# MarvelMathesh/sincformer-metacog-speech-enhancement

Hardware: AMD Instinct MI355X
Metric: audio frames/sec/GPU (16 kHz, 512-frame utts) + mask RMSE vs CPU ref (higher is better)
Workload: dtype fp16 MFMA operands (PerceptionAgent, fusion, Conformer GEMMs, heads) + bf16 attention core, fp32 accumulate (ops.POLICIES['mixed']); 1 GPU; B256 x 512-frame utterances (L40880, T512) forward; batch_per_gpu=256, samples=40880, frames_per_utt=512, launch=eager launches, streams=2, precision_policy=mixed

## Files before the change

sincformer_metacog_speech_enhancement_amd/csrc/conv16p.hip:

```cpp
#include "gemm16_epi.h"

struct ConvPParams {
  Gemm2Params g;
  Gemm2Params gs;
  const u16* x1; const float* sc1; const float* sh1;
  const u16* x2; const float* sc2; const float* sh2;
  int Lin, Cin, pad, nMt;
  long long x_batch_stride;
};

__device__ __forceinline__ float gelu_as(float z) {
  const float ax = fabsf(z) * 0.70710678118654752440f;
  const float t = __builtin_amdgcn_rcpf(1.0f + 0.3275911f * ax);
  const float ex = __builtin_amdgcn_exp2f(-0.72134752044448170368f * z * z);
  const float poly = t * (0.254829592f + t * (-0.284496736f + t * (1.421413741f + t * (-1.453152027f + t * 1.061405429f))));
  const float erfa = 1.0f - poly * ex;
  return z * (0.5f + 0.5f * copysignf(erfa, z));
}

typedef _Float16 h2_t __attribute__((ext_vector_type(2)));
__device__ __forceinline__ uint32_t gelu_as_h2p(uint32_t zb) {
  const h2_t z = __builtin_bit_cast(h2_t, zb);
  const h2_t az = __builtin_bit_cast(h2_t, zb & 0x7fff7fffu);
  const h2_t u = az * (h2_t)(_Float16)(0.3275911f * 0.70710678118654752440f) + (h2_t)(_Float16)1.0f;
  h2_t t;
  t[0] = __builtin_amdgcn_rcph(u[0]);
  t[1] = __builtin_amdgcn_rcph(u[1]);
  const h2_t ex = __builtin_elementwise_exp2(z * z * (h2_t)(_Float16)(-0.72134752044448170368f));
  h2_t poly = t * (_Float16)1.061405429f + (_Float16)(-1.453152027f);
  poly = poly * t + (_Float16)1.421413741f;
  poly = poly * t + (_Float16)(-0.284496736f);
  poly = poly * t + (_Float16)0.254829592f;
  poly = poly * t;
  const h2_t erfa = (h2_t)(_Float16)1.0f - poly * ex;
  const h2_t sg = __builtin_bit_cast(h2_t, (__builtin_bit_cast(uint32_t, erfa) & 0x7fff7fffu) | (zb & 0x80008000u));
  return __builtin_bit_cast(uint32_t, z * (sg * (_Float16)0.5f + (_Float16)0.5f));
}

template <class T, bool FULL>
__device__ __forceinline__ void convp_epilogue_impl(const Gemm2Params& g, f32x16 (&acc)[2][2], unsigned char* img, const float* bias_s,
                                                    int lane, int b, int colb, int row_base) {
  constexpr int ROWB = 144;
  const int l31 = lane & 31, hl = lane >> 5;
  float ps[2][4], pq[2][4];
#pragma unroll
  for (int j = 0; j < 2; ++j)
#pragma unroll
    for (int gq = 0; gq < 4; ++gq) {
      const int n0 = colb + j * 32 + 8 * gq + 4 * hl;
      const f32x4 bv = *reinterpret_cast<const f32x4*>(bias_s + n0);
      float s_ = 0.f, q_ = 0.f;
#pragma unroll
      for (int i = 0; i < 2; ++i) {
        const bool rowok = FULL || (row_base + i * 32 + l31 < g.Lout);
#pragma unroll
        for (int e = 0; e < 4; ++e) {
          const float v = acc[i][j][4 * gq + e] + bv[e];
          acc[i][j][4 * gq + e] = v;
          if (rowok) {
            s_ += v;
            q_ = __builtin_fmaf(v, v, q_);
          }
        }
      }
      ps[j][gq] = s_;
      pq[j][gq] = q_;
    }
  if (g.gn_partial) {
    const int cpg = g.gn_group >> 3;
    const int ngroups = g.N / g.gn_group;
    float v16[16];
#pragma unroll
    for (int j = 0; j < 2; ++j)
#pragma unroll
      for (int gq = 0; gq < 4; ++gq) {
        v16[j * 4 + gq] = ps[j][gq];
        v16[8 + j * 4 + gq] = pq[j][gq];
      }
    float tot = wave_sum16_transpose(v16, lane);
    if (cpg >= 2) tot += dpp_perm<0xB1>(tot);
    if (cpg == 4) tot += dpp_perm<0x4E>(tot);
    const int gq_ = lane & 3, j_ = (lane >> 2) & 1, stat = (lane >> 3) & 1;
    if (lane < 16 && (gq_ & (cpg - 1)) == 0 && (row_base >> 6) < g.gn_slots) {
      const long long sl = ((long long)b * g.gn_slots + (row_base >> 6)) * ngroups + (colb + j_ * 32 + 8 * gq_) / g.gn_group;
      g.gn_partial[sl * 2 + stat] = tot;
    }
  }
  const int osz = g.out_f32 == 1 ? 4 : 2;
  auto ors = __builtin_amdgcn_make_buffer_rsrc((void*)(reinterpret_cast<unsigned char*>(g.out) + (long long)b * g.o_batch_stride * osz), 0,
                                               g.Lout * g.ldo * osz, 0x00020000);
  if (g.out_f32 != 1) {
    __builtin_amdgcn_s_waitcnt(0xC07F);
    __builtin_amdgcn_wave_barrier();
#define CONVP_PACK_IMG(PK)                                                                                             \
  _Pragma("unroll") for (int i = 0; i < 2; ++i)                                                                        \
  _Pragma("unroll") for (int j = 0; j < 2; ++j)                                                                        \
  _Pragma("unroll") for (int gq = 0; gq < 4; ++gq) {                                                                   \
    u32x2 w;                                                                                                           \
    w[0] = PK(acc[i][j][4 * gq + 0], acc[i][j][4 * gq + 1]);                                                           \
    w[1] = PK(acc[i][j][4 * gq + 2], acc[i][j][4 * gq + 3]);                                                           \
    *reinterpret_cast<u32x2*>(img + (i * 32 + l31) * ROWB + (j * 32 + 8 * gq + 4 * hl) * 2) = w;                       \
  }
    if ((g.out_f32 == 2) == (T::id == SFM_DT_BF16)) { CONVP_PACK_IMG(F16::pack) } else { CONVP_PACK_IMG(BF16::pack) }
#undef CONVP_PACK_IMG
    __builtin_amdgcn_s_waitcnt(0xC07F);
    __builtin_amdgcn_wave_barrier();
    u32x4 rv[8];
#pragma unroll
    for (int k = 0; k < 8; ++k) {
      const int c = lane + 64 * k;
      rv[k] = *reinterpret_cast<const u32x4*>(img + (c >> 3) * ROWB + (c & 7) * 16);
    }
#pragma unroll
    for (int k = 0; k < 8; ++k) {
      const int c = lane + 64 * k;
      const int row = c >> 3, ch = c & 7;
      __builtin_amdgcn_raw_buffer_store_b128(rv[k], ors, ((row_base + row) * g.ldo + colb + ch * 8) * 2, 0, 0);
    }
  } else {
#pragma unroll
    for (int i = 0; i < 2; ++i) {
      __builtin_amdgcn_s_waitcnt(0xC07F);
      __builtin_amdgcn_wave_barrier();
#pragma unroll
      for (int j = 0; j < 2; ++j)
#pragma unroll
        for (int gq = 0; gq < 4; ++gq)
          *reinterpret_cast<f32x4*>(img + l31 * 272 + (j * 32 + 8 * gq + 4 * hl) * 4) =
              f32x4{acc[i][j][4 * gq + 0], acc[i][j][4 * gq + 1], acc[i][j][4 * gq + 2], acc[i][j][4 * gq + 3]};
      __builtin_amdgcn_s_waitcnt(0xC07F);
      __builtin_amdgcn_wave_barrier();
#pragma unroll
      for (int k = 0; k < 8; ++k) {
        const int c = lane + 64 * k;
        const int row = c >> 4, ch = c & 15;
        const u32x4 v = *reinterpret_cast<const u32x4*>(img + row * 272 + ch * 16);
        __builtin_amdgcn_raw_buffer_store_b128(v, ors, ((row_base + i * 32 + row) * g.ldo + colb + ch * 4) * 4, 0, 0);
      }
    }
  }
}

template <class T>
__device__ __forceinline__ void convp_epilogue(const Gemm2Params& g, f32x16 (&acc)[2][2], unsigned char* img, const float* bias_s,
                                               int lane, int b, int colb, int row_base) {
  if (row_base + 64 <= g.Lout) convp_epilogue_impl<T, true>(g, acc, img, bias_s, lane, b, colb, row_base);
  else convp_epilogue_impl<T, false>(g, acc, img, bias_s, lane, b, colb, row_base);
}

template <class T, int KS, int STRIDE, int NPASS, bool SKIP, bool TWO_IN>
__global__ __launch_bounds__(256, 2) void conv16p_kernel(ConvPParams p) {
  constexpr int R = 127 * STRIDE + KS;
  constexpr int PLANES = (STRIDE == 2 && KS > 1) ? 2 : 1;
  constexpr int PR = (((STRIDE == 2) ? (R + 1) / 2 : R) + 7) / 8 * 8;
  constexpr int PATCH = PLANES * PR * 128;
  constexpr int WT = 128 * 128;
  constexpr int TPS = NPASS * KS + (SKIP ? 1 : 0);
  static_assert(!SKIP || NPASS == 1, "the fused skip conv needs N = 128");
  static_assert(PATCH + 2 * WT >= 4 * 9216, "epilogue images fit in the patch + ring area");
  extern __shared__ __attribute__((aligned(16))) unsigned char smem[];
  unsigned char* ring = smem + PATCH;
  constexpr int RING = (TWO_IN && PATCH > 2 * WT) ? PATCH : 2 * WT;
  float* bias_s = reinterpret_cast<float*>(smem + PATCH + RING);

  const int tid = threadIdx.x, lane = tid & 63;
  const int wave = __builtin_amdgcn_readfirstlane(tid >> 6);
  const int wm = wave >> 1, wn = wave & 1;
  const int l31 = lane & 31, hl = lane >> 5;

  for (int i = tid; i < NPASS * 128; i += 256) bias_s[i] = p.g.bias ? p.g.bias[i] : 0.f;
  if (SKIP && tid < 128) bias_s[256 + tid] = p.gs.bias ? p.gs.bias[tid] : 0.f;
  int id = blockIdx.x;
  {
    const int total = gridDim.x, q = total >> 3, r = total & 7, xcd = id & 7, slot = id >> 3;
    id = (xcd < r ? xcd * (q + 1) : r * (q + 1) + (xcd - r) * q) + slot;
  }
  const int mtile = id % p.nMt, b = id / p.nMt;
  const int l0 = mtile * 128;
  const int nslab = p.Cin >> 6;
  const int Q = nslab * TPS;

  auto w_rs = __builtin_amdgcn_make_buffer_rsrc((void*)p.g.W, 0, p.g.w_records, 0x00020000);
  auto ws_rs = __builtin_amdgcn_make_buffer_rsrc((void*)(SKIP ? p.gs.W : p.g.W), 0, SKIP ? p.gs.w_records : p.g.w_records, 0x00020000);
  int b_row[4], b_swz[4];
#pragma unroll
  for (int i = 0; i < 4; ++i) {
    b_row[i] = (wave * 4 + i) * 8 + (lane >> 3);
    b_swz[i] = ((lane & 7) ^ ((b_row[i] >> 1) & 7)) * 8;
  }
  auto issue_w = [&](int q) {
    const int slab = q / TPS, j = q - slab * TPS;
    unsigned char* dst = ring + (q & 1) * WT;
    if (SKIP && j == TPS - 1) {
#pragma unroll
      for (int i = 0; i < 4; ++i)
        __builtin_amdgcn_raw_ptr_buffer_load_lds(ws_rs, (lds_ptr_t)(dst + (wave * 4 + i) * 1024), 16,
                                                 (b_row[i] * p.gs.Kpad + slab * 64 + b_swz[i]) * 2, 0, 0, 0);
    } else {
      const int np = j / KS, t = j - np * KS;
      const int koff = t * p.Cin + slab * 64;
#pragma unroll
      for (int i = 0; i < 4; ++i)
        __builtin_amdgcn_raw_ptr_buffer_load_lds(w_rs, (lds_ptr_t)(dst + (wave * 4 + i) * 1024), 16,
                                                 ((np * 128 + b_row[i]) * p.g.Kpad + koff + b_swz[i]) * 2, 0, 0, 0);
    }
  };

  f32x16 acc[NPASS][2][2], accs[2][2];
#pragma unroll
  for (int n = 0; n < NPASS; ++n)
#pragma unroll
    for (int i = 0; i < 2; ++i)
#pragma unroll
      for (int j = 0; j < 2; ++j)
#pragma unroll
        for (int r = 0; r < 16; ++r) acc[n][i][j][r] = 0.f;
#pragma unroll
  for (int i = 0; i < 2; ++i)
#pragma unroll
    for (int j = 0; j < 2; ++j)
#pragma unroll
      for (int r = 0; r < 16; ++r) accs[i][j][r] = 0.f;

  int fb_off[2][4];
#pragma unroll
  for (int j = 0; j < 2; ++j) {
    const int row = wn * 64 + j * 32 + l31;
#pragma unroll
    for (int s = 0; s < 4; ++s) fb_off[j][s] = row * 128 + (((2 * s + hl) ^ ((row >> 1) & 7)) << 4);
  }

  constexpr int JSTEP = (PLANES == 1 && STRIDE == 2) ? 2 : 1;
  constexpr int LROWS = PLANES * PR;
  constexpr int NPIECE = (LROWS + 7) / 8;
  auto x1_rs = __builtin_amdgcn_make_buffer_rsrc((void*)(p.x1 + (long long)b * p.x_batch_stride), 0, p.Lin * p.Cin * 2, 0x00020000);
  auto x2_rs = __builtin_amdgcn_make_buffer_rsrc((void*)((TWO_IN ? p.x2 : p.x1) + (long long)b * p.x_batch_stride), 0,
                                                 p.Lin * p.Cin * 2, 0x00020000);
  auto row_pos = [&](int lr) {
    const int plane = (PLANES == 2) ? (lr >= PR ? 1 : 0) : 0;
    const int idx = lr - plane * PR;
    const int j = (PLANES == 2) ? 2 * idx + plane : idx * JSTEP;
    const int pos = l0 * STRIDE - p.pad + j;
    return (lr < LROWS && j < R && pos >= 0 && pos < p.Lin) ? pos : -1;
  };
  const int sp_ = tid & 7, srow = tid >> 3;
  const int sc_ = sp_ ^ ((srow >> 1) & 7);
  auto stage_patch = [&](int slab) {
    for (int pc = wave; pc < NPIECE; pc += 4) {
      const int lr = pc * 8 + (lane >> 3);
      const int pos = row_pos(lr);
      const int c = (lane & 7) ^ ((lr >> 1) & 7);
      const int voff = pos >= 0 ? (pos * p.Cin + slab * 64 + c * 8) * 2 : -1;
      __builtin_amdgcn_raw_ptr_buffer_load_lds(x1_rs, (lds_ptr_t)(smem + pc * 1024), 16, voff, 0, 0, 0);
      if (TWO_IN) __builtin_amdgcn_raw_ptr_buffer_load_lds(x2_rs, (lds_ptr_t)(ring + pc * 1024), 16, voff, 0, 0, 0);
    }
    const int ch0 = slab * 64 + sc_ * 8;
    float a1[8], d1[8], a2[8];
    {
      const f32x4* ps = reinterpret_cast<const f32x4*>(p.sc1 + (long long)b * p.Cin + ch0);
      const f32x4* ph = reinterpret_cast<const f32x4*>(p.sh1 + (long long)b * p.Cin + ch0);
      const f32x4 s0 = ps[0], s1 = ps[1], h0 = ph[0], h1 = ph[1];
#pragma unroll
      for (int e = 0; e < 4; ++e) { a1[e] = s0[e]; a1[4 + e] = s1[e]; d1[e] = h0[e]; d1[4 + e] = h1[e]; }
      if (TWO_IN) {
        const f32x4* qs = reinterpret_cast<const f32x4*>(p.sc2 + (long long)b * p.Cin + ch0);
        const f32x4* qh = reinterpret_cast<const f32x4*>(p.sh2 + (long long)b * p.Cin + ch0);
        const f32x4 t0 = qs[0], t1 = qs[1], g0 = qh[0], g1 = qh[1];
#pragma unroll
        for (int e = 0; e < 4; ++e) { a2[e] = t0[e]; a2[4 + e] = t1[e]; d1[e] += g0[e]; d1[4 + e] += g1[e]; }
      }
    }
    wait_vmcnt<0>();
    __syncthreads();
#pragma unroll 2
    for (int lr = srow; lr < LROWS; lr += 32) {
      if (row_pos(lr) < 0) continue;
      unsigned char* q1 = smem + lr * 128 + sp_ * 16;
      const u32x4 v1 = *reinterpret_cast<const u32x4*>(q1);
      u32x4 v2 = {0u, 0u, 0u, 0u};
      if (TWO_IN) v2 = *reinterpret_cast<const u32x4*>(ring + lr * 128 + sp_ * 16);
      u32x4 o;
#pragma unroll
      for (int e = 0; e < 4; ++e) {
        if (T::id == SFM_DT_F16) {
          uint32_t zpk;
          float t0 = d1[2 * e], t1 = d1[2 * e + 1];
          if (TWO_IN) {
            asm("v_fma_mix_f32 %0, %1, %2, %3 op_sel:[0,0,0] op_sel_hi:[1,0,0]" : "=v"(t0) : "v"(v2[e]), "v"(a2[2 * e]), "v"(d1[2 * e]));
            asm("v_fma_mix_f32 %0, %1, %2, %3 op_sel:[1,0,0] op_sel_hi:[1,0,0]" : "=v"(t1) : "v"(v2[e]), "v"(a2[2 * e + 1]), "v"(d1[2 * e + 1]));
          }
          asm("v_fma_mixlo_f16 %0, %1, %2, %3 op_sel:[0,0,0] op_sel_hi:[1,0,0]\n\t"
              "v_fma_mixhi_f16 %0, %1, %4, %5 op_sel:[1,0,0] op_sel_hi:[1,0,0]"
              : "=&v"(zpk) : "v"(v1[e]), "v"(a1[2 * e]), "v"(t0), "v"(a1[2 * e + 1]), "v"(t1));
          o[e] = gelu_as_h2p(zpk);
          continue;
        }
        float z0 = T::to_f32((u16)(v1[e] & 0xffffu)) * a1[2 * e] + d1[2 * e];
        float z1 = T::to_f32((u16)(v1[e] >> 16)) * a1[2 * e + 1] + d1[2 * e + 1];
        if (TWO_IN) {
          z0 += T::to_f32((u16)(v2[e] & 0xffffu)) * a2[2 * e];
          z1 += T::to_f32((u16)(v2[e] >> 16)) * a2[2 * e + 1];
        }
        o[e] = pack2<T>(gelu_as(z0), gelu_as(z1));
      }
      *reinterpret_cast<u32x4*>(q1) = o;
    }
  };

  auto mma_tile = [&](int q, int t, f32x16 (&a)[2][2]) {
    const unsigned char* wb = ring + (q & 1) * WT;
    int arow[2];
#pragma unroll
    for (int i = 0; i < 2; ++i) {
      const int rw = wm * 64 + i * 32 + l31;
      arow[i] = (PLANES == 2) ? (t & 1) * PR + rw + (t >> 1) : ((STRIDE == 2) ? rw : rw + t);
    }
#pragma unroll
    for (int s = 0; s < 4; ++s) {
      u32x4 fa[2], fb[2];
#pragma unroll
      for (int i = 0; i < 2; ++i)
        fa[i] = *reinterpret_cast<const u32x4*>(smem + arow[i] * 128 + (((2 * s + hl) ^ ((arow[i] >> 1) & 7)) << 4));
#pragma unroll
      for (int j = 0; j < 2; ++j) fb[j] = *reinterpret_cast<const u32x4*>(wb + fb_off[j][s]);
#pragma unroll
      for (int i = 0; i < 2; ++i)
#pragma unroll
        for (int j = 0; j < 2; ++j) a[i][j] = T::mfma(fb[j], fa[i], a[i][j]);
    }
  };

  if (!TWO_IN) issue_w(0);
  for (int slab = 0; slab < nslab; ++slab) {
    if (slab > 0) __syncthreads();
    stage_patch(slab);
    __syncthreads();
    const int q0 = slab * TPS;
    if (TWO_IN) issue_w(q0);
#pragma unroll
    for (int j = 0; j < TPS; ++j) {
      const int q = q0 + j;
      wait_ring<0>();
      __builtin_amdgcn_s_barrier();
      if (j + 1 < TPS) issue_w(q + 1);
      if (SKIP && j == TPS - 1) {
        mma_tile(q, p.pad, accs);
      } else {
        const int np = j / KS, t = j - np * KS;
        if (np == 0) mma_tile(q, t, acc[0]);
        else mma_tile(q, t, acc[NPASS - 1]);
      }
      if (j + 1 == TPS && !TWO_IN && q + 1 < Q) issue_w(q + 1);
    }
  }
  __syncthreads();
  unsigned char* img = smem + wave * 9216;
#pragma unroll
  for (int n = 0; n < NPASS; ++n) convp_epilogue<T>(p.g, acc[n], img, bias_s, lane, b, n * 128 + wn * 64, l0 + wm * 64);
  if (SKIP) convp_epilogue<T>(p.gs, accs, img, bias_s + 256, lane, b, wn * 64, l0 + wm * 64);
}

template <class T, int KS, int STRIDE, int NPASS, bool SKIP, bool TWO_IN>
static int launch_convp(const ConvPParams& p, hipStream_t stream) {
  constexpr int R = 127 * STRIDE + KS;
  constexpr int PLANES = (STRIDE == 2 && KS > 1) ? 2 : 1;
  constexpr int PR = (((STRIDE == 2) ? (R + 1) / 2 : R) + 7) / 8 * 8;
  constexpr int patch = PLANES * PR * 128;
  constexpr int lds = patch + ((TWO_IN && patch > 2 * 128 * 128) ? patch : 2 * 128 * 128) + 384 * 4;
  SFM_LAUNCH_LDS((conv16p_kernel<T, KS, STRIDE, NPASS, SKIP, TWO_IN>), dim3(p.nMt * p.g.B), dim3(256), lds, stream, p);
  return SFM_OK;
}

static void convp_fill(Gemm2Params& g, const void* W, const float* bias, void* out, float* gn_partial, int B, int Lout, int N,
                       int Kpad, int out_f32, int gn_group) {
  g = Gemm2Params{};
  g.W = (const u16*)W; g.bias = bias; g.out = out; g.gn_partial = gn_partial;
  g.B = B; g.Lout = Lout; g.N = N; g.Npad = N; g.K = Kpad; g.Kpad = Kpad; g.ldo = N; g.o_batch_stride = (long long)Lout * N;
  g.alpha = 1.0f; g.epi = EPI_NONE; g.out_f32 = out_f32; g.gn_group = gn_group; g.nsplit = 0;
  g.w_records = (int)((long long)N * Kpad * 2);
  g.gn_slots = 2 * ((Lout + 127) / 128);
  const int osz = out_f32 == 1 ? 4 : 2;
  g.vec_ok = ((((uintptr_t)out) % 16) == 0 && ((N * osz) % 16) == 0) ? 1 : 0;
  g.p_drop = 0.f; g.seed = 0u; g.aux = nullptr; g.out2 = nullptr; g.resid = nullptr;
}

extern "C" int sfm_conv16p(const void* x1, const float* sc1, const float* sh1, const void* x2, const float* sc2, const float* sh2,
                           const void* W, const float* bias, void* out, float* gn_partial, const void* Ws, const float* bias_s,
                           void* out_s, float* gn_partial_s, int B, int Lin, int Cin, int N, int ksize, int stride, int pad,
                           int out_f32, int gn_group, int dtype, void* stream) {
  if (!x1 || !sc1 || !sh1 || !W || !out) return SFM_ERR_ARG;
  if ((x2 != nullptr) != (sc2 != nullptr) || (x2 != nullptr) != (sh2 != nullptr)) return SFM_ERR_ARG;
  if (B <= 0 || Lin <= 0 || Cin <= 0 || (Cin % 64) != 0 || (N != 128 && N != 256)) return SFM_ERR_SHAPE;
  if (out_f32 < 0 || out_f32 > 2) return SFM_ERR_SHAPE;
  if (gn_partial && gn_group != 8 && gn_group != 16 && gn_group != 32) return SFM_ERR_SHAPE;
  if ((long long)Lin * Cin * 2 >= (1LL << 31) || (long long)N * ksize * Cin * 2 >= (1LL << 31)) return SFM_ERR_SHAPE;
  if ((long long)((Lin + 2 * pad - ksize) / stride + 1) * N * 4 >= (1LL << 31)) return SFM_ERR_SHAPE;
  const int Lout = (Lin + 2 * pad - ksize) / stride + 1;
  if (Lout <= 0) return SFM_ERR_SHAPE;
  const bool skip = Ws != nullptr;
  if (skip && (!out_s || N != 128 || ksize != 7 || stride != 2)) return SFM_ERR_SHAPE;
  if ((((uintptr_t)out) % 16) != 0 || (out_s && (((uintptr_t)out_s) % 16) != 0)) return SFM_ERR_SHAPE;
  ConvPParams p{};
  convp_fill(p.g, W, bias, out, gn_partial, B, Lout, N, ksize * Cin, out_f32, gn_group);
  if (skip) convp_fill(p.gs, Ws, bias_s, out_s, gn_partial_s, B, Lout, N, Cin, out_f32, gn_group);
  p.x1 = (const u16*)x1; p.sc1 = sc1; p.sh1 = sh1; p.x2 = (const u16*)x2; p.sc2 = sc2; p.sh2 = sh2;
  p.Lin = Lin; p.Cin = Cin; p.pad = pad; p.nMt = (Lout + 127) / 128; p.x_batch_stride = (long long)Lin * Cin;
  hipStream_t st = (hipStream_t)stream;
  const bool two = x2 != nullptr;
  const int key = ksize * 100 + stride * 10 + pad;
#define CONVP_GO(TT)                                                                                       \
  if (key == 723 && N == 128 && skip) return two ? launch_convp<TT, 7, 2, 1, true, true>(p, st) : launch_convp<TT, 7, 2, 1, true, false>(p, st); \
  if (key == 723 && N == 256 && !skip && two) return launch_convp<TT, 7, 2, 2, false, true>(p, st);        \
  if (key == 311 && N == 128 && !two) return launch_convp<TT, 3, 1, 1, false, false>(p, st);                \
  if (key == 311 && N == 256 && !two) return launch_convp<TT, 3, 1, 2, false, false>(p, st);                \
  if (key == 522 && N == 256 && two) return launch_convp<TT, 5, 2, 2, false, true>(p, st);                  \
  if (key == 120 && N == 256 && two) return launch_convp<TT, 1, 2, 2, false, true>(p, st);
  if (dtype == SFM_DT_BF16) { CONVP_GO(BF16) }
  if (dtype == SFM_DT_F16) { CONVP_GO(F16) }
#undef CONVP_GO
  return SFM_ERR_SHAPE;
}
```

sincformer_metacog_speech_enhancement_amd/csrc/sfm_common.h:

```cpp
#pragma once
#include <hip/hip_runtime.h>
#include <stdint.h>
#include <atomic>
#include <mutex>
#include "sincformer_hip.h"

typedef uint16_t u16;
typedef __attribute__((ext_vector_type(4))) float f32x4;
typedef __attribute__((ext_vector_type(16))) float f32x16;
typedef __attribute__((ext_vector_type(8))) __bf16 bf16x8_t;
typedef __attribute__((ext_vector_type(8))) _Float16 f16x8_t;
typedef __attribute__((ext_vector_type(4))) short s16x4;
typedef __attribute__((ext_vector_type(4))) uint32_t u32x4;
typedef __attribute__((ext_vector_type(2))) uint32_t u32x2;
typedef __attribute__((ext_vector_type(2))) float f32x2;
typedef __attribute__((ext_vector_type(2))) __bf16 bf16x2_t;
typedef __attribute__((ext_vector_type(2))) _Float16 f16x2_t;

struct BF16 {
  static constexpr int id = SFM_DT_BF16;
  static __device__ __forceinline__ u16 from_f32(float f) {
    __bf16 h = (__bf16)f;
    return __builtin_bit_cast(u16, h);
  }
  static __device__ __forceinline__ float to_f32(u16 b) {
    return __builtin_bit_cast(float, (uint32_t)b << 16);
  }
  static __device__ __forceinline__ uint32_t pack(float lo, float hi) {
    f32x2 v = {lo, hi};
    return __builtin_bit_cast(uint32_t, __builtin_convertvector(v, bf16x2_t));
  }
  static __device__ __forceinline__ f32x16 mfma(u32x4 a, u32x4 b, f32x16 c) {
    return __builtin_amdgcn_mfma_f32_32x32x16_bf16(__builtin_bit_cast(bf16x8_t, a),
                                                   __builtin_bit_cast(bf16x8_t, b), c, 0, 0, 0);
  }
  static __device__ __forceinline__ f32x4 mfma16(u32x4 a, u32x4 b, f32x4 c) {
    return __builtin_amdgcn_mfma_f32_16x16x32_bf16(__builtin_bit_cast(bf16x8_t, a),
                                                   __builtin_bit_cast(bf16x8_t, b), c, 0, 0, 0);
  }
};

struct F16 {
  static constexpr int id = SFM_DT_F16;
  static __device__ __forceinline__ u16 from_f32(float f) {
    _Float16 h = (_Float16)f;
    return __builtin_bit_cast(u16, h);
  }
  static __device__ __forceinline__ float to_f32(u16 b) {
    return (float)__builtin_bit_cast(_Float16, b);
  }
  static __device__ __forceinline__ uint32_t pack(float lo, float hi) {
    f32x2 v = {lo, hi};
    return __builtin_bit_cast(uint32_t, __builtin_convertvector(v, f16x2_t));
  }
  static __device__ __forceinline__ f32x16 mfma(u32x4 a, u32x4 b, f32x16 c) {
    return __builtin_amdgcn_mfma_f32_32x32x16_f16(__builtin_bit_cast(f16x8_t, a),
                                                  __builtin_bit_cast(f16x8_t, b), c, 0, 0, 0);
  }
  static __device__ __forceinline__ f32x4 mfma16(u32x4 a, u32x4 b, f32x4 c) {
    return __builtin_amdgcn_mfma_f32_16x16x32_f16(__builtin_bit_cast(f16x8_t, a),
                                                  __builtin_bit_cast(f16x8_t, b), c, 0, 0, 0);
  }
};

template <class T>
__device__ __forceinline__ uint32_t pack2(float lo, float hi) {
  return T::pack(lo, hi);
}
template <class T>
__device__ __forceinline__ uint32_t pack2_out(float lo, float hi, bool other) {
  if (T::id == SFM_DT_BF16) return other ? F16::pack(lo, hi) : BF16::pack(lo, hi);
  return other ? BF16::pack(lo, hi) : F16::pack(lo, hi);
}

__device__ __forceinline__ uint32_t sfm_hash(uint32_t seed, unsigned long long idx) {
  uint32_t x = (uint32_t)idx * 0x9E3779B1u ^ (uint32_t)(idx >> 32) * 0x85EBCA77u ^ seed;
  x ^= x >> 16; x *= 0x7FEB352Du; x ^= x >> 15; x *= 0x846CA68Bu; x ^= x >> 16;
  return x;
}
__device__ __forceinline__ uint32_t sfm_keep_threshold(float p) { return (uint32_t)ceilf(p * 16777216.0f); }
__device__ __forceinline__ float sfm_keep_from_group(uint32_t gh, uint32_t j, uint32_t thr24, float inv_keep) {
  uint32_t x = gh + j * 0x9E3779B1u;
  x ^= x >> 15; x *= 0x846CA68Bu; x ^= x >> 16;
  return ((x >> 8) >= thr24) ? inv_keep : 0.f;
}
__device__ __forceinline__ uint32_t sfm_keep_word24(uint32_t gh, uint32_t j) {
  uint32_t x = gh + j * 0x9E3779B1u;
  x ^= x >> 15; x *= 0x846CA68Bu; x ^= x >> 16;
  return x >> 8;
}
__device__ __forceinline__ float sfm_keep_scale(uint32_t seed, unsigned long long idx, float p, float inv_keep) {
  return sfm_keep_from_group(sfm_hash(seed, idx >> 3), (uint32_t)(idx & 7ull), sfm_keep_threshold(p), inv_keep);
}
__device__ __forceinline__ void sfm_keep_scale8(uint32_t seed, unsigned long long e0, float p, float inv_keep, float (&k)[8]) {
  if (e0 & 7ull) {
#pragma unroll
    for (int i = 0; i < 8; ++i) k[i] = sfm_keep_scale(seed, e0 + i, p, inv_keep);
    return;
  }
  const uint32_t gh = sfm_hash(seed, e0 >> 3), thr = sfm_keep_threshold(p);
#pragma unroll
  for (int i = 0; i < 8; ++i) k[i] = sfm_keep_from_group(gh, (uint32_t)i, thr, inv_keep);
}


__device__ __forceinline__ int mfma_row(int r, int lane) { return (r & 3) + 8 * (r >> 2) + 4 * (lane >> 5); }

__device__ __forceinline__ float gelu_erf(float x) { return 0.5f * x * (1.0f + erff(x * 0.70710678118654752440f)); }
__device__ __forceinline__ float normal_cdf_poly(float z) {
  const float zc = __builtin_amdgcn_fmed3f(z, -3.75f, 3.75f);
  const float u = zc * zc;
  float q = 3.912424329e-08f;
  q = fmaf(q, u, -2.376248530e-06f);
  q = fmaf(q, u, 6.234773063e-05f);
  q = fmaf(q, u, -9.441793120e-04f);
  q = fmaf(q, u, 9.362551949e-03f);
  q = fmaf(q, u, -6.578987097e-02f);
  q = fmaf(q, u, 3.987064729e-01f);
  return fmaf(zc, q, 0.5f);
}
__device__ __forceinline__ float sigmoid_f(float x) { return 1.0f / (1.0f + __expf(-x)); }
__device__ __forceinline__ float swish_f(float x) { return x * sigmoid_f(x); }

__device__ __forceinline__ float wave_sum(float v) {
#pragma unroll
  for (int o = 32; o > 0; o >>= 1) v += __shfl_xor(v, o, 64);
  return v;
}
__device__ __forceinline__ float wave_max(float v) {
#pragma unroll
  for (int o = 32; o > 0; o >>= 1) v = fmaxf(v, __shfl_xor(v, o, 64));
  return v;
}
__device__ __forceinline__ double wave_sum_d(double v) {
#pragma unroll
  for (int o = 32; o > 0; o >>= 1) v += __shfl_xor(v, o, 64);
  return v;
}

template <int CTRL>
__device__ __forceinline__ float dpp_perm(float v) {
  return __builtin_bit_cast(float, __builtin_amdgcn_update_dpp(0, __builtin_bit_cast(int, v), CTRL, 0xF, 0xF, false));
}
template <int CTRL>
__device__ __forceinline__ float dpp_perm_add(float v) {
  return v + dpp_perm<CTRL>(v);
}
__device__ __forceinline__ float wave_sum_dpp(float v) {
  v = dpp_perm_add<0xB1>(v);
  v = dpp_perm_add<0x4E>(v);
  v = dpp_perm_add<0x141>(v);
  v = dpp_perm_add<0x140>(v);
  const int iv = __builtin_bit_cast(int, v);
  const float r0 = __builtin_bit_cast(float, __builtin_amdgcn_readlane(iv, 0));
  const float r1 = __builtin_bit_cast(float, __builtin_amdgcn_readlane(iv, 16));
  const float r2 = __builtin_bit_cast(float, __builtin_amdgcn_readlane(iv, 32));
  const float r3 = __builtin_bit_cast(float, __builtin_amdgcn_readlane(iv, 48));
  return (r0 + r1) + (r2 + r3);
}

__device__ __forceinline__ void xhalf_swap(float v, float& lo, float& hi) {
  uint32_t a = __builtin_bit_cast(uint32_t, v), c = a;
  asm volatile("s_nop 1\n\tv_permlane32_swap_b32 %0, %1" : "+v"(a), "+v"(c));
  lo = __builtin_bit_cast(float, a);
  hi = __builtin_bit_cast(float, c);
}
__device__ __forceinline__ float xhalf_max(float v) {
  float lo, hi;
  xhalf_swap(v, lo, hi);
  return fmaxf(lo, hi);
}
__device__ __forceinline__ float xhalf_sum(float v) {
  float lo, hi;
  xhalf_swap(v, lo, hi);
  return lo + hi;
}

__device__ __forceinline__ float wave_sum16_transpose(const float (&v)[16], int lane) {
  const bool b3 = lane & 8, b2 = lane & 4, b1 = lane & 2, b0 = lane & 1;
  float w[8], x[4], y[2];
#pragma unroll
  for (int i = 0; i < 8; ++i) w[i] = (b3 ? v[i + 8] : v[i]) + dpp_perm<0x140>(b3 ? v[i] : v[i + 8]);
#pragma unroll
  for (int i = 0; i < 4; ++i) x[i] = (b2 ? w[i + 4] : w[i]) + dpp_perm<0x141>(b2 ? w[i] : w[i + 4]);
#pragma unroll
  for (int i = 0; i < 2; ++i) y[i] = (b1 ? x[i + 2] : x[i]) + dpp_perm<0x4E>(b1 ? x[i] : x[i + 2]);
  float z = (b0 ? y[1] : y[0]) + dpp_perm<0xB1>(b0 ? y[0] : y[1]);
  float a = z, c = z;
  asm volatile("s_nop 1\n\tv_permlane16_swap_b32 %0, %1" : "+v"(a), "+v"(c));
  return xhalf_sum(a + c);
}

typedef __attribute__((address_space(3))) void* lds_ptr_t;

template <int N>
__device__ __forceinline__ void wait_vmcnt() {
  asm volatile("s_waitcnt vmcnt(%0)" ::"n"(N) : "memory");
}
template <int N>
__device__ __forceinline__ void wait_ring() {
  asm volatile("s_waitcnt vmcnt(%0) lgkmcnt(0)" ::"n"(N) : "memory");
}
__device__ __forceinline__ void ring_barrier() {
  asm volatile("s_waitcnt lgkmcnt(0)" ::: "memory");
  __builtin_amdgcn_s_barrier();
  asm volatile("" ::: "memory");
}
__device__ __forceinline__ void frag_read(u32x4& dst, uint32_t lds_addr) {
  asm volatile("ds_read_b128 %0, %1" : "=v"(dst) : "v"(lds_addr) : "memory");
}
template <int N>
__device__ __forceinline__ void frag_wait(u32x4& frag) {
  asm volatile("s_waitcnt lgkmcnt(%1)" : "+v"(frag) : "n"(N) : "memory");
}

__device__ __forceinline__ int sfm_seg_find(const int* __restrict__ off, int n, int r) {
  int lo = 0, hi = n;
  while (hi - lo > 1) {
    const int mid = (lo + hi) >> 1;
    if (off[mid] <= r) lo = mid;
    else hi = mid;
  }
  return lo;
}

#define SFM_LAUNCH(kernel, grid, block, shmem, stream, ...)                    \
  do {                                                                         \
    (void)hipGetLastError();                                                   \
    hipLaunchKernelGGL(kernel, grid, block, shmem, stream, __VA_ARGS__);       \
    if (hipGetLastError() != hipSuccess) return SFM_ERR_LAUNCH;                \
  } while (0)

static inline int sfm_device(int* dev) {
  return (hipGetDevice(dev) == hipSuccess && *dev >= 0 && *dev < 64) ? SFM_OK : SFM_ERR_LAUNCH;
}
template <auto Kernel>
static int sfm_grant_lds(int bytes) {
  static std::atomic<int> granted[64];
  static std::mutex raise;
  int dev = 0;
  if (sfm_device(&dev) != SFM_OK) return SFM_ERR_LAUNCH;
  if (bytes <= granted[dev].load(std::memory_order_acquire)) return SFM_OK;
  std::lock_guard<std::mutex> lock(raise);
  if (bytes <= granted[dev].load(std::memory_order_relaxed)) return SFM_OK;
  if (hipFuncSetAttribute((const void*)Kernel, hipFuncAttributeMaxDynamicSharedMemorySize, bytes) != hipSuccess)
    return SFM_ERR_LAUNCH;
  granted[dev].store(bytes, std::memory_order_release);
  return SFM_OK;
}
#define SFM_LAUNCH_LDS(kernel, grid, block, shmem, stream, ...)                \
  do {                                                                         \
    if (sfm_grant_lds<kernel>(shmem) != SFM_OK) return SFM_ERR_LAUNCH;         \
    SFM_LAUNCH(kernel, grid, block, shmem, stream, __VA_ARGS__);               \
  } while (0)

inline int sfm_cu_count() {
  static std::atomic<int> ncu[64];
  int dev = 0;
  if (sfm_device(&dev) != SFM_OK) return 0;
  int n = ncu[dev].load(std::memory_order_relaxed);
  if (n == 0) {
    hipDeviceProp_t prop;
    if (hipGetDeviceProperties(&prop, dev) != hipSuccess) return 0;
    n = prop.multiProcessorCount > 0 ? prop.multiProcessorCount : 256;
    ncu[dev].store(n, std::memory_order_relaxed);
  }
  return n;
}

static inline long long sfm_capped_blocks(long long n, int per, long long cap) {
  const long long nb = (n + per - 1) / per;
  return nb > cap ? cap : nb;
}

int sfm_fold_partials(float* ws, float* out, long long rows, int cols, long long ldo, int S, int accumulate, void* stream);
int sfm_fold_partials2(float* ws, float* out, float* out2, int cols1, int cols, int S, int accumulate, void* stream);
int sfm_fold_partials_f64(double* ws, double* out, long long rows, int cols, long long ldo, int S, int accumulate, void* stream);
```

Measured before the change: 9.085 million STFT frames/s (whole job).

## Software-pipeline LDS fragment reads in conv16p with precomputed addresses and immediate offsets

Replaces the mma_tile lambda with a compile-time unrolled tap loop. It uses inline-asm ds_read_b128 with immediate offsets and precomputed per-lane LDS base addresses, using XOR to pick the swizzle slot. Fragments for the next k-step, and for the next tap, are double-buffered and prefetched while MFMAs run, with fine-grained lgkmcnt waits. The aim is to hide LDS latency and cut address arithmetic. The cost is more registers for the double buffers and fragile hand-counted waitcnt values.

```diff
diff --git a/sincformer_metacog_speech_enhancement_amd/csrc/conv16p.hip b/sincformer_metacog_speech_enhancement_amd/csrc/conv16p.hip
--- a/sincformer_metacog_speech_enhancement_amd/csrc/conv16p.hip
+++ b/sincformer_metacog_speech_enhancement_amd/csrc/conv16p.hip
@@ -1,4 +1,14 @@
 #include "gemm16_epi.h"
+#include <utility>
+
+template <class F, int... Is>
+__device__ __forceinline__ void static_for_seq(F&& f, std::integer_sequence<int, Is...>) {
+  (f(std::integral_constant<int, Is>{}), ...);
+}
+template <int N, class F>
+__device__ __forceinline__ void static_for(F&& f) {
+  static_for_seq(f, std::make_integer_sequence<int, N>{});
+}
 
 struct ConvPParams {
   Gemm2Params g;
@@ -158,7 +168,7 @@
   constexpr int TPS = NPASS * KS + (SKIP ? 1 : 0);
   static_assert(!SKIP || NPASS == 1, "the fused skip conv needs N = 128");
   static_assert(PATCH + 2 * WT >= 4 * 9216, "epilogue images fit in the patch + ring area");
-  extern __shared__ __attribute__((aligned(16))) unsigned char smem[];
+  extern __shared__ __attribute__((aligned(128))) unsigned char smem[];
   unsigned char* ring = smem + PATCH;
   constexpr int RING = (TWO_IN && PATCH > 2 * WT) ? PATCH : 2 * WT;
   float* bias_s = reinterpret_cast<float*>(smem + PATCH + RING);
@@ -222,12 +232,18 @@
 #pragma unroll
       for (int r = 0; r < 16; ++r) accs[i][j][r] = 0.f;
 
-  int fb_off[2][4];
-#pragma unroll
-  for (int j = 0; j < 2; ++j) {
-    const int row = wn * 64 + j * 32 + l31;
-#pragma unroll
-    for (int s = 0; s < 4; ++s) fb_off[j][s] = row * 128 + (((2 * s + hl) ^ ((row >> 1) & 7)) << 4);
+  const uint32_t lds0 = (uint32_t)(uintptr_t)(lds_ptr_t)smem;
+  constexpr int NSHIFT = (PLANES == 2) ? (KS + 1) / 2 : ((STRIDE == 2) ? 1 : KS);
+  uint32_t w_addr[4], p_addr[NSHIFT];
+  {
+    const int w_row = wn * 64 + l31;
+#pragma unroll
+    for (int s = 0; s < 4; ++s) w_addr[s] = lds0 + (uint32_t)(PATCH + w_row * 128 + (((2 * s + hl) ^ ((w_row >> 1) & 7)) << 4));
+#pragma unroll
+    for (int sh = 0; sh < NSHIFT; ++sh) {
+      const int ar = wm * 64 + l31 + sh;
+      p_addr[sh] = lds0 + (uint32_t)(ar * 128 + ((hl ^ ((ar >> 1) & 7)) << 4));
+    }
   }
 
   constexpr int JSTEP = (PLANES == 1 && STRIDE == 2) ? 2 : 1;
@@ -307,28 +323,17 @@
     }
   };
 
-  auto mma_tile = [&](int q, int t, f32x16 (&a)[2][2]) {
-    const unsigned char* wb = ring + (q & 1) * WT;
-    int arow[2];
-#pragma unroll
-    for (int i = 0; i < 2; ++i) {
-      const int rw = wm * 64 + i * 32 + l31;
-      arow[i] = (PLANES == 2) ? (t & 1) * PR + rw + (t >> 1) : ((STRIDE == 2) ? rw : rw + t);
-    }
-#pragma unroll
-    for (int s = 0; s < 4; ++s) {
-      u32x4 fa[2], fb[2];
-#pragma unroll
-      for (int i = 0; i < 2; ++i)
-        fa[i] = *reinterpret_cast<const u32x4*>(smem + arow[i] * 128 + (((2 * s + hl) ^ ((arow[i] >> 1) & 7)) << 4));
-#pragma unroll
-      for (int j = 0; j < 2; ++j) fb[j] = *reinterpret_cast<const u32x4*>(wb + fb_off[j][s]);
-#pragma unroll
-      for (int i = 0; i < 2; ++i)
-#pragma unroll
-        for (int j = 0; j < 2; ++j) a[i][j] = T::mfma(fb[j], fa[i], a[i][j]);
-    }
-  };
+  u32x4 fa[2][2], fb[2][2];
+#pragma unroll
+  for (int e = 0; e < 2; ++e)
+#pragma unroll
+    for (int i = 0; i < 2; ++i) fa[e][i] = fb[e][i] = u32x4{0u, 0u, 0u, 0u};
+  static_assert(PLANES == 1 || ((PR >> 1) & 3) == 0, "plane 1's swizzle is an XOR of plane 0's");
+  constexpr auto tile_tap = [](int j) { return (SKIP && j == TPS - 1) ? KS / 2 : j % KS; };
+  constexpr auto tap_shift = [](int t) { return (PLANES == 2) ? (t >> 1) : ((STRIDE == 2) ? 0 : t); };
+  constexpr auto tap_off = [](int t) { return (PLANES == 2) ? (t & 1) * PR * 128 : 0; };
+  constexpr auto tap_xor = [](int t) { return (PLANES == 2 && (t & 1)) ? ((PR >> 1) & 7) << 4 : 0; };
+  constexpr bool SLOT_CT = (TPS % 2) == 0;
 
   if (!TWO_IN) issue_w(0);
   for (int slab = 0; slab < nslab; ++slab) {
@@ -337,21 +342,56 @@
     __syncthreads();
     const int q0 = slab * TPS;
     if (TWO_IN) issue_w(q0);
-#pragma unroll
-    for (int j = 0; j < TPS; ++j) {
-      const int q = q0 + j;
+    {
+      constexpr int T0 = tile_tap(0);
+      const uint32_t pa = p_addr[tap_shift(T0)] ^ (uint32_t)tap_xor(T0);
+      frag_read_at<tap_off(T0)>(fa[0][0], pa);
+      frag_read_at<tap_off(T0) + 4096>(fa[0][1], pa);
+    }
+    static_for<TPS>([&](auto jc) {
+      constexpr int J = decltype(jc)::value;
+      constexpr bool SK = SKIP && J == TPS - 1;
+      constexpr bool MORE = J + 1 < TPS;
+      constexpr int TAP = tile_tap(J), POFF = tap_off(TAP), PXOR = tap_xor(TAP);
+      constexpr int WOFF = SLOT_CT ? (J & 1) * WT : 0;
+      f32x16 (&a)[2][2] = *(SK ? &accs : &acc[SK ? 0 : J / KS]);
+      const int q = q0 + J;
+      const uint32_t w_slot = SLOT_CT ? 0u : (uint32_t)((q & 1) * WT);
+      uint32_t pb = p_addr[tap_shift(TAP)];
+      asm volatile("" : "+v"(pb));
       wait_ring<0>();
       __builtin_amdgcn_s_barrier();
-      if (j + 1 < TPS) issue_w(q + 1);
-      if (SKIP && j == TPS - 1) {
-        mma_tile(q, p.pad, accs);
-      } else {
-        const int np = j / KS, t = j - np * KS;
-        if (np == 0) mma_tile(q, t, acc[0]);
-        else mma_tile(q, t, acc[NPASS - 1]);
-      }
-      if (j + 1 == TPS && !TWO_IN && q + 1 < Q) issue_w(q + 1);
-    }
+      if constexpr (MORE) issue_w(q + 1);
+      frag_read_at<WOFF>(fb[0][0], w_addr[0] + w_slot);
+      frag_read_at<WOFF + 4096>(fb[0][1], w_addr[0] + w_slot);
+      static_for<4>([&](auto sc) {
+        constexpr int S = decltype(sc)::value;
+        constexpr int NEXT = S < 3 ? 4 : (MORE ? 2 : 0);
+        u32x4 (&ca)[2] = fa[S & 1], (&cb)[2] = fb[S & 1], (&na)[2] = fa[(S + 1) & 1], (&nb)[2] = fb[(S + 1) & 1];
+        if constexpr (S < 3) {
+          const uint32_t pa = pb ^ (uint32_t)(((S + 1) << 5) ^ PXOR), wa = w_addr[S + 1] + w_slot;
+          frag_read_at<POFF>(na[0], pa);
+          frag_read_at<WOFF>(nb[0], wa);
+          frag_read_at<WOFF + 4096>(nb[1], wa);
+          frag_read_at<POFF + 4096>(na[1], pa);
+        } else if constexpr (MORE) {
+          constexpr int T1 = tile_tap(J + 1);
+          const uint32_t pa = p_addr[tap_shift(T1)] ^ (uint32_t)tap_xor(T1);
+          frag_read_at<tap_off(T1)>(na[0], pa);
+          frag_read_at<tap_off(T1) + 4096>(na[1], pa);
+        }
+        if constexpr (S == 0) frag_wait<1 + NEXT>(cb[0], ca[0]);
+        else frag_wait<2 + NEXT>(ca[0], cb[0]);
+        a[0][0] = T::mfma(cb[0], ca[0], a[0][0]);
+        if constexpr (S == 0) frag_wait<NEXT>(cb[1], ca[1]);
+        else frag_wait<1 + NEXT>(cb[1]);
+        a[0][1] = T::mfma(cb[1], ca[0], a[0][1]);
+        if constexpr (S != 0) frag_wait<NEXT>(ca[1]);
+        a[1][0] = T::mfma(cb[0], ca[1], a[1][0]);
+        a[1][1] = T::mfma(cb[1], ca[1], a[1][1]);
+      });
+    });
+    if (!TWO_IN && q0 + TPS < Q) issue_w(q0 + TPS);
   }
   __syncthreads();
   unsigned char* img = smem + wave * 9216;
diff --git a/sincformer_metacog_speech_enhancement_amd/csrc/sfm_common.h b/sincformer_metacog_speech_enhancement_amd/csrc/sfm_common.h
--- a/sincformer_metacog_speech_enhancement_amd/csrc/sfm_common.h
+++ b/sincformer_metacog_speech_enhancement_amd/csrc/sfm_common.h
@@ -212,6 +212,15 @@
 template <int N>
 __device__ __forceinline__ void frag_wait(u32x4& frag) {
   asm volatile("s_waitcnt lgkmcnt(%1)" : "+v"(frag) : "n"(N) : "memory");
+}
+template <int N>
+__device__ __forceinline__ void frag_wait(u32x4& f0, u32x4& f1) {
+  asm volatile("s_waitcnt lgkmcnt(%2)" : "+v"(f0), "+v"(f1) : "n"(N) : "memory");
+}
+template <int OFF>
+__device__ __forceinline__ void frag_read_at(u32x4& dst, uint32_t lds_addr) {
+  static_assert(OFF >= 0 && OFF < 65536, "ds_read offset field");
+  asm volatile("ds_read_b128 %0, %1 offset:%2" : "+v"(dst) : "v"(lds_addr), "n"(OFF) : "memory");
 }
 
 __device__ __forceinline__ int sfm_seg_find(const int* __restrict__ off, int n, int r) {
```

Result: no change. 9.132 million STFT frames/s (whole job), median of 6 (+0.5%).
